# hasnainfarid/Mujoco_Gymnasium_Environments

Hardware: AMD Instinct MI355X
Metric: env steps/sec (whole node), humanoid_soccer 4096 envs/GPU at 1/2/4/8 MI355X (higher is better)
Workload: dtype f64

## Files before the change

### mujoco_gymnasium_environments_amd/csrc/mgx_api.hip

```cpp
#include <hip/hip_runtime.h>

#include <cmath>
#include <cstdio>
#include <cstring>
#include <map>
#include <mutex>
#include <string>
#include <vector>

#include "mgx_internal.h"

using namespace mgx;

MGX_PROF_SETTER(mgx_prof_set_buffer)

namespace {
thread_local std::string g_err;
int fail(int code, const std::string& msg) {
  g_err = msg;
  return code;
}
#define HIPCHK(x) MGX_HIPCHK(x)
}

// ... 493 lines not shown
  return pgs_lanes() == 64 ? a / 2 : a;
}

static int wide_arena_bytes(const mgx_model* m) {
  const int wide_lds = m->hooks.pgs_wide_lds;
  const int rb = m->precision == MGX_F32 ? 4 : 8;
  const int nv = m->precision == MGX_F32 ? m->mf.nv : m->md.nv;
  const int maxE = m->Ls.max_nefc;
  const int nbRun = (maxE / 4 + MGX_PGS_RING_LDS - 1) / MGX_PGS_RING_LDS * MGX_PGS_RING_LDS;
  const int nbA = nbRun + MGX_PGS_RING_LDS - 1;
  const int bcap = 32 + (maxE / 4) * (8 + 32 * ((nv + 7) / 8));
  const int worst = nbA * (4 * MGX_SCAL * rb + 4 * mgx_twl(false)) + ((bcap + 3) & ~3) * rb;
  return wide_lds && pgs_lanes() == 16 && worst + 64 <= 160 * 1024 ? (worst + 15) & ~15 : 0;
}

size_t mgx::make_staged_pipe(const mgx_model* m, void* ws, int n_env, int banks, Pipe* P, bool rk, int nobs) {
  int rb = m->precision == MGX_F32 ? 4 : 8;
  int nq = m->precision == MGX_F32 ? m->mf.nq : m->md.nq;
  int nv = m->precision == MGX_F32 ? m->mf.nv : m->md.nv;
  Pipe p{};
  p.base = (char*)ws;
  p.N = n_env; p.R = banks; p.S = n_env * (1 + banks);
  p.maxE = m->Ls.max_nefc; p.nv = nv; p.dpl = (nv + 7) / 8;
  const Hooks& H = m->hooks;
  const bool cap_env = H.pgs_lds_rows > 0;
  int capE = cap_env ? (H.pgs_lds_rows + 3) / 4 * 4 : MGX_PGS_LDS_ROWS;
  if (capE < 4 || capE > p.maxE) capE = MGX_PGS_LDS_ROWS;
  if (rk) {
    capE = H.rk_lds_rows > 0 ? (H.rk_lds_rows + 3) / 4 * 4 : 256;
    if (capE < 4) capE = 256;
  }
// ... 18 lines not shown
  p.bcap = 32 + (p.maxE / 4) * (8 + 32 * ((nv + 7) / 8));
  p.tw = MGX_TW;
  p.nobs = nobs;
  size_t off = 0;
  auto take = [&](size_t bytes) { size_t r = off; off = (off + bytes + 255) / 256 * 256; return r; };
  size_t S = (size_t)p.S, NB = (size_t)n_env * (banks > 0 ? banks : 1);
  p.o_ctr = take(64);
  p.o_carry = take(S * p.carry_stride * rb);
  p.o_carryi = take(S * p.carryi_stride * 4);
  p.o_ne = take(S * 4); p.o_blen = take(S * 4); p.o_niter = take(S * 4); p.o_k2list = take(S * 4); p.o_k2big = take(S * 4); p.o_fix = take((size_t)n_env * 4);
  p.hmain = !rk && !cap_env && !p.sqg && !H.pgs_lds_b && p.capE < p.maxE &&
            staged_pgs_lds_bytes(m, p.maxE, pgs_lanes(), 1, mgx_twl(false)) <=
                (H.pgs_wpc == 4 ? staged_pgs_lds_bytes(m, p.capE, pgs_lanes(), 0, mgx_twl(false))
                                : 160 * 1024 / H.pgs_wpc);
  if (p.hmain) p.warena = 0;
  p.prio_rows = H.pgs_prio_rows > 0 ? H.pgs_prio_rows : p.capE;
  p.nbk = (p.hmain ? p.maxE : p.capE) / 4 + 1;
  p.o_hist = take((size_t)(p.maxE / 4 + 1) * 4);
  p.o_blist = take((size_t)(p.maxE / 4 + 1) * S * 4);
  p.o_scal = take(S * p.maxE * MGX_SCAL * rb);
  p.o_blk = take(S * (p.maxE / 4) * p.tw * 4);
  p.o_B = take(S * (size_t)p.bcap * rb);
  p.o_vout = take(S * 64 * rb);
  p.o_bq = take(NB * nq * rb); p.o_bv = take(NB * nv * rb); p.o_ba = take(NB * nv * rb); p.o_btime = take(NB * rb);
  p.o_bobs = take(NB * nobs * 4); p.o_bprev = take(NB * 6 * rb); p.o_bwind = take(NB * 3 * rb);
  p.o_bk = take(NB * 4); p.o_bep = take(NB * 4); p.o_bwarn = take(NB * 4); p.o_bseed = take(NB * 8);
  int nb = m->precision == MGX_F32 ? m->mf.nbody : m->md.nbody;
  p.maxC = m->Ls.max_ncon;
  p.o_cpos = take(S * 3 * (size_t)p.maxC * rb);
  p.o_tq = take(nq * rb); p.o_tv = take(nv * rb); p.o_ta = take(64 * rb); p.o_tt = take(rb);
  p.o_tx = take(3 * nb * rb); p.o_txq = take(4 * nb * rb); p.o_tsc = take(3 * nb * rb); p.o_tn = take(4);
  p.o_tcg = take(2 * p.maxC * 4); p.o_tcd = take(p.maxC * rb); p.o_tcm = take(p.maxC * rb);
  p.o_rkw = take(S * 4);
  p.o_tscr = take(m->L.gB ? (size_t)m->L.gB_stride * rb : 64);
  if (rk) {
    const int nq4 = (nq + 3) & ~3;
    p.rk_stride = 2 * nq4 + 8 * 64 + 4;
    p.o_rk = take(S * p.rk_stride * rb);
    p.o_rks = take(S * 4);
  }
  if (P) *P = p;
  return off;
}
static size_t make_pipe(const mgx_model* m, void* ws, int n_env, int banks, Pipe* P) {
  return make_staged_pipe(m, ws, n_env, banks, P, false, 80);
}

int mgx::staged_pgs_lds_bytes(const mgx_model* m, int rows, int lps, int sqg, int twl) {
  int rb = m->precision == MGX_F32 ? 4 : 8;
  int nb3 = (rows / 4 + MGX_PGS_RING - 1) / MGX_PGS_RING * MGX_PGS_RING;
  const int spw = 64 / lps;
  const int sq = sqg ? 4 : 4 * MGX_SCAL;
  return spw * (sq * nb3 + 4) * rb + spw * nb3 * 4 * twl + 64;
}
static int pgs_lds_bytes(const mgx_model* m, int rows, int sqg = 0) {
  return staged_pgs_lds_bytes(m, rows, pgs_lanes(), sqg, mgx_twl(false));
}

mgx::Hooks mgx::read_hooks() {
  Hooks h;
  auto get = [](const char* name, int dflt) {
    const char* v = getenv(name);
    return v && *v ? atoi(v) : dflt;
  };
  h.pgs_lds_rows = get("MGX_PGS_LDS_ROWS", 0);
  h.rk_lds_rows = get("MGX_RK_LDS_ROWS", 0);
  h.pgs_single = get("MGX_PGS_SINGLE", 0);
  h.pgs_lds_b = get("MGX_PGS_LDS_B", MGX_PGS_LDS_B) != 0;
  h.pgs_arena = get("MGX_PGS_ARENA", 0);
  h.pgs_lds_pad = get("MGX_PGS_LDS_PAD", 0);
  h.pgs_wide_lds = get("MGX_PGS_WIDE_LDS", 1);
  h.pgs_spw = get("MGX_PGS_SPW", 0);
  h.pgs_prio_rows = get("MGX_PGS_PRIO_ROWS", 0);
  h.tight_bp = get("MGX_TIGHT_BROADPHASE", -1);
  h.pgs_wpc = get("MGX_PGS_WPC", 4);
  if (h.pgs_wpc < 4 || h.pgs_wpc > 16) h.pgs_wpc = 4;
  h.side_stream = get("MGX_SIDE_STREAM", 1) != 0;
  h.gcon = get("MGX_GCON", 1);
  h.rows_lds = get("MGX_ROWS_LDS", 0);
  return h;
}

struct SideStream {
  hipStream_t s;
  hipEvent_t rows, big;
};
static SideStream* side_stream(hipStream_t st) {
  static std::mutex mu;
// ... 28 lines not shown
                              float* obs, double* reward, uint8_t* terminated, uint8_t* truncated, float* final_obs,
                              int autoreset, uint64_t seed, int env_offset, int n_env, const uint8_t* mask,
                              hipStream_t st) {
  Pipe P;
  int banks = autoreset ? e->banks : 0;
  size_t need = make_pipe(m, e->workspace, n_env, e->banks, &P);
  if (e->workspace_bytes < need) return fail(MGX_E_ARG, "workspace smaller than mgx_soccer_workspace_bytes");
  int slots = n_env * (1 + banks);
  const Hooks& H = m->hooks;
  const int rlds = H.rows_lds > m->Ls.bytes && H.rows_lds <= 64 * 1024 ? H.rows_lds : m->Ls.bytes;
  launch_soccer_rows<T>(Ms, ids, *s, *e, action, n_env, mask, P, banks, slots, rlds, st);
  T scale = (T)1 / (M.meaninertia * (T)(M.nv > 1 ? M.nv : 1));
  const int wgrid = 64 / pgs_lanes() * MGX_PGS_WIDE_GRID, wlds = pgs_lds_bytes(m, P.maxE);
  int mlds = H.pgs_lds_b ? P.arena : pgs_lds_bytes(m, P.capE, P.sqg);
  if (P.hmain) mlds = std::max(mlds, pgs_lds_bytes(m, P.maxE, 1));
  if (H.pgs_lds_pad > mlds && H.pgs_lds_pad <= 96 * 1024) mlds = H.pgs_lds_pad;
  if (!H.pgs_lds_b && (P.maxE <= P.capE || P.hmain)) {
    launch_pgs<T>(P, slots, mlds, st, M.iterations, M.tolerance, scale, 0, H);
  } else if (SideStream* side = (!H.pgs_lds_b && H.side_stream) ? side_stream(st) : nullptr) {
    HIPCHK(hipEventRecord(side->rows, st));
    HIPCHK(hipStreamWaitEvent(side->s, side->rows, 0));
    launch_pgs<T>(P, wgrid, wlds, side->s, M.iterations, M.tolerance, scale, 1, H);
    HIPCHK(hipEventRecord(side->big, side->s));
    launch_pgs<T>(P, slots, mlds, st, M.iterations, M.tolerance, scale, 0, H);
    HIPCHK(hipStreamWaitEvent(st, side->big, 0));
  } else {
    launch_pgs<T>(P, slots, mlds, st, M.iterations, M.tolerance, scale, 0, H);
    launch_pgs<T>(P, wgrid, wlds, st, M.iterations, M.tolerance, scale, 1, H);
  }
  launch_soccer_finish<T>(Mf, ids, *s, *e, action, obs, reward, terminated, truncated, final_obs, autoreset, seed,
                          env_offset, n_env, mask, P, banks, m->Lf.bytes, st);
  int fgrid = n_env < 256 ? n_env : 256;
// ... 304 lines not shown
```

### mujoco_gymnasium_environments_amd/csrc/mgx_internal.h

```cpp
#pragma once
#include <hip/hip_runtime.h>

#include <string>

#include "../../include/mgx.h"
#include "mgx_bipedal.h"
#include "mgx_construction.h"
#include "mgx_dancing.h"
#include "mgx_martial.h"
#include "mgx_parkour.h"
#include "mgx_staged.h"

namespace mgx {
struct Hooks {
  int pgs_lds_rows = 0;
  int rk_lds_rows = 0;
  int pgs_single = 0;
  int pgs_lds_b = 0;
  int pgs_arena = 0;
  int pgs_lds_pad = 0;
  int pgs_wide_lds = 1;
  int pgs_spw = 0;
  int pgs_wpc = 4;
  int pgs_prio_rows = 0;
  int tight_bp = -1;
  int side_stream = 1;
  int gcon = 1;
  int rows_lds = 0;
};
Hooks read_hooks();
struct RayState;
struct SensorState;
}

struct mgx_model {
  mgx::Hooks hooks;
  int precision;
  int device;
  void* dbuf = nullptr;
// ... 58 lines not shown
template <typename T>
void launch_soccer_rows(const DevModel<T>& Ms, const SoccerIds<T>& ids, const mgx_state& s, const mgx_soccer_env& ev,
                        const float* action, int n_env, const uint8_t* mask, const Pipe& P, int banks, int slots, int lds,
                        hipStream_t st);
template <typename T>
void launch_soccer_finish(const DevModel<T>& Mf, const SoccerIds<T>& ids, const mgx_state& s, const mgx_soccer_env& ev,
                          const float* action, float* obs, double* reward, uint8_t* terminated, uint8_t* truncated,
                          float* final_obs, int autoreset, uint64_t seed, int env_offset, int n_env, const uint8_t* mask,
                          const Pipe& P, int banks, int lds, hipStream_t st);
template <typename T>
void launch_soccer_settle(const DevModel<T>& Ms, const DevModel<T>& Mf, const SoccerIds<T>& ids, const mgx_state& s,
                          const mgx_soccer_env& ev, const T* draws, float* obs, uint64_t seed, int env_offset, int n_env,
                          const uint8_t* mask, const Pipe& P, int mode, int grid, int lds, hipStream_t st, int maxit, T tol,
                          T scale);
int staged_kernels_configure(int precision, int ls, int lf, int settle);
size_t make_staged_pipe(const mgx_model* m, void* ws, int n_env, int banks, Pipe* P, bool rk, int nobs);
int staged_pgs_lds_bytes(const mgx_model* m, int rows, int lps, int sqg, int twl);
int bipedal_staged_configure(const mgx_model* m);
int bipedal_step_staged(const mgx_model* m, const mgx_state* s, const mgx_bipedal_env* e, const float* action, float* obs,
                        double* reward, uint8_t* terminated, uint8_t* truncated, float* final_obs, int autoreset,
                        uint64_t seed, int env_offset, int n_env, const uint8_t* mask, hipStream_t st);
int bipedal_reset_staged(const mgx_model* m, const mgx_state* s, const mgx_bipedal_env* e, const void* draws,
                         float* obs, uint64_t seed, int env_offset, int n_env, const uint8_t* mask, hipStream_t st);
int64_t bipedal_workspace_bytes(const mgx_model* m, int n_env, int banks);
int bipedal_workspace_init(const mgx_model* m, void* workspace, uint64_t bytes, int n_env, int banks, hipStream_t st);
bool parkour_staged_ok(const mgx_model* m);
int parkour_staged_configure(const mgx_model* m);
int parkour_step_staged(const mgx_model* m, const mgx_state* s, const mgx_parkour_env* e, const float* action, float* obs,
                        double* reward, uint8_t* terminated, uint8_t* truncated, float* final_obs, int autoreset,
                        uint64_t seed, int env_offset, int n_env, const uint8_t* mask, hipStream_t st);
int parkour_reset_staged(const mgx_model* m, const mgx_state* s, const mgx_parkour_env* e, const void* draws,
// ... 24 lines not shown
```

### mujoco_gymnasium_environments_amd/csrc/mgx_pk_staged.hip

```cpp
#include "mgx_internal.h"

using namespace mgx;

namespace mgx {

constexpr int PK_LPS = 16;
constexpr int PK_OBS = 95;
enum { PK_SETTLE_RESET = 0, PK_SETTLE_FIXUP = 1 };
enum { PK_SUBSTEPS = 10 };

template <typename T>
__device__ __forceinline__ void pk_bank_init_draws(const DevModel<T>& m, Env<T>& e, const ParkourIds<T>& ids,
                                                   const Pipe& P, int bi, int episode, uint64_t seed, T d0, T d1) {
  const int l = lane_id();
  reset_env(m, e);
  if (l == 0) {
    e.qpos[0] = (T)2.0; e.qpos[1] = (T)0.0; e.qpos[2] = (T)0.6;
    e.qpos[3] = (T)1; e.qpos[4] = 0; e.qpos[5] = 0; e.qpos[6] = 0;
    e.qpos[ids.platform_qpos] = d0;
    e.qpos[ids.pendulum_qpos] = d1;
  }
  wsync();
  copy_g(P.at<T>(P.o_bq) + (size_t)bi * m.nq, e.qpos, m.nq);
  if (l < m.nv) {
// ... 302 lines not shown
#define MGX_PK_EPL(EPL_VAR, CALL) \
  switch (EPL_VAR) {              \
    case 1: { constexpr int E = 1; CALL; } break; \
    case 2: { constexpr int E = 2; CALL; } break; \
    case 3: { constexpr int E = 3; CALL; } break; \
    default: { constexpr int E = 4; CALL; } break; \
  }

template <typename T>
int step_staged(const mgx_model* m, const DevModel<T>& M, const DevModel<T>& Ms, const DevModel<T>& Mf,
                const ParkourIds<T>& ids, const mgx_state* s, const mgx_parkour_env* e, const float* action,
                float* obs, double* reward, uint8_t* terminated, uint8_t* truncated, float* final_obs, int autoreset,
                uint64_t seed, int env_offset, int n_env, const uint8_t* mask, hipStream_t st) {
  Pipe P;
  const int banks = autoreset ? e->banks : 0;
  const size_t need = make_staged_pipe(m, e->workspace, n_env, e->banks, &P, false, PK_OBS);
  if (e->workspace_bytes < need) return fail(MGX_E_ARG, "workspace smaller than mgx_parkour_workspace_bytes");
  const int slots = n_env * (1 + banks);
  const T scale = (T)1 / (M.meaninertia * (T)(M.nv > 1 ? M.nv : 1));
  const int mlds = std::max(staged_pgs_lds_bytes(m, P.capE, PK_LPS, 0, 8),
                           P.hmain ? staged_pgs_lds_bytes(m, P.maxE, PK_LPS, 1, 8) : 0);
  const int spw = 64 / PK_LPS, grid = (slots + spw - 1) / spw;
  for (int k = 0; k < PK_SUBSTEPS; k++) {
    hipLaunchKernelGGL(k_pk_rows<T>, dim3(slots), dim3(64), m->Ls.bytes, st, Ms, ids, *s, action, e->action_f64, n_env,
                       mask, P, banks, k);
    MGX_PK_EPL(pk_epl(M), hipLaunchKernelGGL((k_pgs_groups<T, E, PK_LPS, false>), dim3(grid), dim3(64), mlds, st, P,
                                             M.iterations, M.tolerance, scale, spw, 0));
    if (banks && P.R > 0)
      hipLaunchKernelGGL(k_pk_bank_finish<T>, dim3(n_env * P.R), dim3(64), m->Lf.bytes, st, Mf, ids, n_env, P);
    hipLaunchKernelGGL(k_pk_finish<T>, dim3(n_env), dim3(64), m->Lf.bytes, st, Mf, ids, *s, *e, action, obs, reward,
                       terminated, truncated, final_obs, autoreset, seed, env_offset, n_env, mask, P, banks, k);
  }
  const int fgrid = n_env < 256 ? n_env : 256;
  MGX_PK_EPL(pk_epl(M), hipLaunchKernelGGL((k_pk_settle<T, E>), dim3(fgrid), dim3(64), pk_settle_lds(m, P), st, Ms, Mf,
                                           ids, *s, *e, (const T*)nullptr, obs, seed, env_offset, n_env,
                                           (const uint8_t*)nullptr, P, (int)PK_SETTLE_FIXUP, M.iterations, M.tolerance,
                                           scale));
  MGX_HIPCHK(hipGetLastError());
  return MGX_OK;
}

template <typename T>
int reset_staged(const mgx_model* m, const DevModel<T>& M, const DevModel<T>& Ms, const DevModel<T>& Mf,
                 const ParkourIds<T>& ids, const mgx_state* s, const mgx_parkour_env* e, const T* draws, float* obs,
                 uint64_t seed, int env_offset, int n_env, const uint8_t* mask, hipStream_t st) {
  Pipe P;
  const size_t need = make_staged_pipe(m, e->workspace, n_env, e->banks, &P, false, PK_OBS);
  if (e->workspace_bytes < need) return fail(MGX_E_ARG, "workspace smaller than mgx_parkour_workspace_bytes");
  const T scale = (T)1 / (M.meaninertia * (T)(M.nv > 1 ? M.nv : 1));
  MGX_PK_EPL(pk_epl(M), hipLaunchKernelGGL((k_pk_settle<T, E>), dim3(n_env), dim3(64), pk_settle_lds(m, P), st, Ms, Mf,
                                           ids, *s, *e, draws, obs, seed, env_offset, n_env, mask, P,
                                           (int)PK_SETTLE_RESET, M.iterations, M.tolerance, scale));
  MGX_HIPCHK(hipGetLastError());
  return MGX_OK;
}

template <typename T>
int configure_t(const mgx_model* m) {
  Pipe P;
  make_staged_pipe(m, nullptr, 1, 1, &P, false, PK_OBS);
  const int pl = staged_pgs_lds_bytes(m, P.maxE, PK_LPS, 0, 8);
  if (pl > 160 * 1024) return fail(MGX_E_CAPACITY, "staged parkour solver LDS exceeds 160 KiB");
  int rc = mgx_set_lds(k_pk_rows<T>, m->Ls.bytes) | mgx_set_lds(k_pk_finish<T>, m->Lf.bytes) |
           mgx_set_lds(k_pk_bank_finish<T>, m->Lf.bytes) | mgx_set_lds(k_pk_template<T, true>, m->L.bytes) |
           mgx_set_lds(k_pk_template<T, false>, m->L.bytes);
  const int sl = pk_settle_lds(m, P);
#define MGX_PK_SET(E) rc |= mgx_set_lds(k_pk_settle<T, E>, sl) | mgx_set_lds(k_pgs_groups<T, E, PK_LPS, false>, pl);
  MGX_PK_SET(1) MGX_PK_SET(2) MGX_PK_SET(3) MGX_PK_SET(4)
#undef MGX_PK_SET
  return rc;
}

}

namespace mgx {
bool parkour_staged_ok(const mgx_model* m) {
  const int nv = m->precision == MGX_F32 ? m->mf.nv : m->md.nv;
  if (!m->staged_ok || nv > 64 || pgs_lanes() != PK_LPS || m->hooks.pgs_lds_b) return false;
  Pipe P;
  make_staged_pipe(m, nullptr, 1, 1, &P, false, PK_OBS);
  return !P.sqg && (P.maxE <= P.capE || P.hmain);
}

int parkour_staged_configure(const mgx_model* m) {
  if (!parkour_staged_ok(m)) return MGX_OK;
  return m->precision == MGX_F32 ? configure_t<float>(m) : configure_t<double>(m);
}

int parkour_step_staged(const mgx_model* m, const mgx_state* s, const mgx_parkour_env* e, const float* action, float* obs,
                        double* reward, uint8_t* terminated, uint8_t* truncated, float* final_obs, int autoreset,
                        uint64_t seed, int env_offset, int n_env, const uint8_t* mask, hipStream_t st) {
  if (!parkour_staged_ok(m)) return fail(MGX_E_UNSUPPORTED, "staged parkour step: model outside the staged pipeline");
  if (e->banks < 0 || e->banks > 16) return fail(MGX_E_ARG, "banks must be in [0, 16]");
  if (m->precision == MGX_F32)
    return step_staged<float>(m, m->mf, m->mfs, m->mff, m->pkf, s, e, action, obs, reward, terminated, truncated,
                              final_obs, autoreset, seed, env_offset, n_env, mask, st);
// ... 3 lines not shown

int parkour_reset_staged(const mgx_model* m, const mgx_state* s, const mgx_parkour_env* e, const void* draws,
                         float* obs, uint64_t seed, int env_offset, int n_env, const uint8_t* mask, hipStream_t st) {
  if (!parkour_staged_ok(m)) return fail(MGX_E_UNSUPPORTED, "staged parkour step: model outside the staged pipeline");
  if (e->banks < 0 || e->banks > 16) return fail(MGX_E_ARG, "banks must be in [0, 16]");
  if (m->precision == MGX_F32)
    return reset_staged<float>(m, m->mf, m->mfs, m->mff, m->pkf, s, e, (const float*)draws, obs, seed, env_offset,
                               n_env, mask, st);
  return reset_staged<double>(m, m->md, m->mds, m->mdf, m->pkd, s, e, (const double*)draws, obs, seed, env_offset,
                              n_env, mask, st);
}

int64_t parkour_workspace_bytes(const mgx_model* m, int n_env, int banks) {
  if (!m || n_env <= 0 || banks < 0 || banks > 16) return fail(MGX_E_ARG, "bad argument");
  if (!parkour_staged_ok(m)) return fail(MGX_E_UNSUPPORTED, "staged parkour step: model outside the staged pipeline");
  return (int64_t)make_staged_pipe(m, nullptr, n_env, banks, nullptr, false, PK_OBS);
}

int parkour_workspace_init(const mgx_model* m, void* workspace, uint64_t bytes, int n_env, int banks, hipStream_t st) {
  if (!m || !workspace || n_env <= 0 || banks < 0 || banks > 16) return fail(MGX_E_ARG, "bad argument");
  if (!parkour_staged_ok(m)) return fail(MGX_E_UNSUPPORTED, "staged parkour step: model outside the staged pipeline");
  Pipe P;
  const size_t need = make_staged_pipe(m, workspace, n_env, banks, &P, false, PK_OBS);
  if (bytes < need) return fail(MGX_E_ARG, "workspace smaller than mgx_parkour_workspace_bytes");
  MGX_HIPCHK(hipMemsetAsync(workspace, 0, need, st));
  const size_t nb = (size_t)n_env * (banks > 0 ? banks : 1);
  MGX_HIPCHK(hipMemsetAsync(P.base + P.o_bk, 0xFF, nb * 4, st));
  if (m->precision == MGX_F32) {
    if (m->L.gB) hipLaunchKernelGGL((k_pk_template<float, true>), dim3(1), dim3(64), m->L.bytes, st, m->mf, P);
    else hipLaunchKernelGGL((k_pk_template<float, false>), dim3(1), dim3(64), m->L.bytes, st, m->mf, P);
  } else {
    if (m->L.gB) hipLaunchKernelGGL((k_pk_template<double, true>), dim3(1), dim3(64), m->L.bytes, st, m->md, P);
    else hipLaunchKernelGGL((k_pk_template<double, false>), dim3(1), dim3(64), m->L.bytes, st, m->md, P);
  }
  MGX_HIPCHK(hipGetLastError());
  return MGX_OK;
}
}
// ... 1 lines not shown
```

### mujoco_gymnasium_environments_amd/csrc/mgx_staged.h

```cpp
#pragma once
#include "mgx_soccer.h"

namespace mgx {

#define MGX_SCAL 5
#define MGX_SQ(k, i) (4 * (k) + (i))
#define MGX_TW 4
__host__ __device__ constexpr int mgx_twl(bool dofb) { return dofb ? 4 : 8; }
#define MGX_PGS_LPS 16
#define MGX_PGS_LDS_B 0
#define MGX_PGS_RING 2
#define MGX_PGS_RING_LDS 2
#define MGX_PGS_LDS_ROWS 192
#define MGX_PGS_WIDE_GRID 256
#define MGX_PGS_WIDE_LDS_GRID 32
#define MGX_PGS_ARENA_F64 49152
#define MGX_PGS_ARENA_F32 32768
enum { FIX_RESET = 2 };

struct Pipe {
  char* base;
  int N, R, S, maxE, dpl, nv;
  int carry_stride;
  int carryi_stride;
  int bcap;
  int capE;
  int arena;
  int sqg;
  int prio_rows;
  int hmain;
  int warena;
  size_t o_cpos;
  size_t o_carry, o_carryi, o_ne, o_blen, o_niter, o_k2list, o_k2big, o_ctr, o_fix, o_scal, o_blk, o_B, o_vout;
  int nbk;
  size_t o_hist, o_blist;
  size_t o_bq, o_bv, o_ba, o_btime, o_bobs, o_bprev, o_bwind, o_bk, o_bep, o_bwarn, o_bseed;
  size_t o_tq, o_tv, o_ta, o_tt, o_tx, o_txq, o_tsc, o_tn, o_tcg, o_tcd, o_tcm;
  int maxC;
  int tw;
  int nobs;
  int rk_stride;
  size_t o_rk, o_rks, o_rkw, o_tscr;
  template <typename X> __device__ __forceinline__ X* at(size_t off) const { return reinterpret_cast<X*>(base + off); }
  __device__ __forceinline__ int* ctr() const { return at<int>(o_ctr); }
};
// ... 380 lines not shown
  for (int k = l; k < 2 * e.ncon; k += 64) ci[k] = e.con_geom[k];
  int* cx = ci + m.L.carry_ints;
  if (l == 0) {
    cx[0] = e.ncon; cx[1] = ne; cx[2] = e.overflow; cx[3] = warn;
    P.at<int>(P.o_ne)[slot] = ne;
    P.at<int>(P.o_blen)[slot] = boff;
#ifdef MGX_PROFILE
    if (g_mgx_prof && slot < (int)gridDim.x) {
      g_mgx_prof[slot * 32 + 20] += ne;
      g_mgx_prof[slot * 32 + 22] += e.ncon;
      g_mgx_prof[slot * 32 + 23] += 1;
      if ((unsigned long long)ne > g_mgx_prof[slot * 32 + 24]) g_mgx_prof[slot * 32 + 24] = ne;
      g_mgx_prof[slot * 32 + 25] += e.overflow != 0;
    }
#endif
    if (!list_slot) {
    } else if (ne > P.capE && !P.hmain) {
      int idx = atomicAdd(P.ctr() + 2, 1);
      P.at<int>(P.o_k2big)[idx] = slot;
    } else if (ne > 0) {
      int idx = atomicAdd(P.ctr() + 1, 1);
      P.at<int>(P.o_k2list)[idx] = slot;
      const int nb = ne >> 2;
      const int r = atomicAdd(P.at<int>(P.o_hist) + nb, 1);
      P.at<int>(P.o_blist)[(size_t)nb * P.S + r] = slot;
    }
  }
}

template <int CTRL>
__device__ __forceinline__ float dpp_row(float v) {
  return __builtin_bit_cast(float, __builtin_amdgcn_mov_dpp(__builtin_bit_cast(int, v), CTRL, 0xf, 0xf, true));
// ... 57 lines not shown
      t.g[d] = in ? e.x + 8u + 4u * (uint32_t)__popcll(below) : 0u;
    }
  } else {
    const uint32_t* e = bt + 8 * blk;
    t.a = e[0];
#pragma unroll
    for (int d = 0; d < EPL; d++) {
      const int gi = d * (LPS / 8) + (j >> 3);
      t.g[d] = (gi < 7 ? e[1 + gi] : 0u) + 4u * (uint32_t)(j & 7);
    }
  }
}

typedef float mgx_f2 __attribute__((ext_vector_type(2)));

template <typename T, int EPL, int LPS, int FS>
__device__ __forceinline__ void pgs_load_block(PgsBlk<T, EPL>& k, const T* Bsl, const T* sq, const T* fb,
                                               const PgsTab<EPL>& t, int blk, int sblk, int j) {
  typedef typename Vec4T<T>::type V4;
  const V4* pa = reinterpret_cast<const V4*>(Bsl + t.a);
  k.a0 = pa[0];
  k.a1 = pa[1];
#pragma unroll
  for (int d = 0; d < EPL; d++) k.b[d] = *reinterpret_cast<const V4*>(Bsl + t.g[d]);
  const V4* q = reinterpret_cast<const V4*>(sq + 4 * MGX_SCAL * sblk);
  k.qb = q[0];
  k.qf = *reinterpret_cast<const V4*>(fb + FS * blk);
  k.qR = q[2];
  k.qi = q[3];
  k.qh = q[4];
  __builtin_amdgcn_sched_barrier(0);
}
template <typename T, int EPL, int LPS, int FS, bool DOFB>
__device__ __forceinline__ void pgs_load_block(PgsBlk<T, EPL>& k, const T* Bsl, const T* sq, const T* fb,
                                               const uint32_t* bt, int blk, int sblk, int j) {
  PgsTab<EPL> t;
  pgs_load_tab<EPL, LPS, DOFB>(t, bt, blk, j);
  pgs_load_block<T, EPL, LPS, FS>(k, Bsl, sq, fb, t, blk, sblk, j);
}
// ... 18 lines not shown
  }
  d0 = p01.x; d1 = p01.y; d2 = p23.x; d3 = p23.y;
}

template <typename T, int EPL>
__device__ __forceinline__ void pgs_update(const PgsBlk<T, EPL>& k, T (&v)[EPL], T dl0, T dl1, T dl2, T dl3) {
#pragma unroll
  for (int d = 0; d < EPL; d++) {
    T x = fma(dl0, k.b[d].x, v[d]);
    x = fma(dl1, k.b[d].y, x);
    x = fma(dl2, k.b[d].z, x);
    v[d] = fma(dl3, k.b[d].w, x);
  }
}

template <typename T, int EPL, int LPS>
__device__ __forceinline__ void pgs_block(const PgsBlk<T, EPL>& k, T (&v)[EPL], T* fblk, bool ok0, T& impr) {
  typedef typename Vec4T<T>::type V4;
  V4* qf = reinterpret_cast<V4*>(fblk);
  const V4 qb = k.qb, f = k.qf, qR = k.qR, qi = k.qi, qh = k.qh;
  T d0, d1, d2, d3;
  pgs_dots(k, v, d0, d1, d2, d3);
  const T t0 = qb.x + qR.x * f.x, t1 = qb.y + qR.y * f.y;
  const T t2 = qb.z + qR.z * f.z, t3 = qb.w + qR.w * f.w;
  slot_sum4<LPS>(d0, d1, d2, d3);
  T dl0, dl1, dl2, dl3;
  V4 nfv;
#define MGX_PGS_ROW(C, I, DOT, DL)                                \
  {                                                               \
    const T fr = f.C, ai = qi.C, hd = qh.C;                       \
    T res = (DOT) + t##I;                                         \
    T fn = fmax(fr - res * ai, (T)0);                             \
    T delta = fn - fr;                                            \
    T change = delta * (delta * hd + res);                        \
    bool keep = !ok0 || change > (T)1e-10;                        \
    DL = keep ? (T)0 : delta;                                     \
    impr -= keep ? (T)0 : change;                                 \
    nfv.C = keep ? fr : fn;                                       \
  }
  MGX_PGS_ROW(x, 0, d0, dl0)
  MGX_PGS_ROW(y, 1, d1 + k.a0.x * dl0, dl1)
  MGX_PGS_ROW(z, 2, d2 + k.a0.y * dl0 + k.a0.z * dl1, dl2)
  MGX_PGS_ROW(w, 3, d3 + k.a0.w * dl0 + k.a1.x * dl1 + k.a1.y * dl2, dl3)
#undef MGX_PGS_ROW
  if ((lane_id() & (LPS - 1)) == 0) *qf = nfv;
  pgs_update(k, v, dl0, dl1, dl2, dl3);
}

template <typename T, int EPL, int LPS, bool BLDS, bool SQG = false, bool DOFB = false>
__device__ __forceinline__ void pgs_group(const Pipe& P, char* smem, int slot, int capE, int maxit, T tol, T scale,
                                          int spw, int arena = -1) {
  constexpr int RING = BLDS ? MGX_PGS_RING_LDS : MGX_PGS_RING;
  typedef typename Vec4T<T>::type V4;
  constexpr int SPW = 64 / LPS;
  const int l = threadIdx.x, s = l / LPS, j = l % LPS;
  (void)spw;
  const int ne = slot >= 0 ? P.at<int>(P.o_ne)[slot] : 0;
  const int nblk = ne >> 2;
  int nm = nblk;
  nm = max(nm, __shfl_xor(nm, 8));
  nm = max(nm, __shfl_xor(nm, 16));
  nm = max(nm, __shfl_xor(nm, 32));
  int nbMax = __builtin_amdgcn_readfirstlane(nm);
  if (spw < 0) nbMax = capE / 4;
  const int nbRun = (nbMax + RING - 1) / RING * RING;
  const size_t sl = (size_t)(slot >= 0 ? slot : 0);
  const T* gsc = P.at<T>(P.o_scal) + sl * P.maxE * MGX_SCAL;
  constexpr int TWL = mgx_twl(DOFB);
  const uint32_t* gbt = P.at<uint32_t>(P.o_blk) + sl * (P.maxE / 4) * MGX_TW;
  const uint16_t* gbt16 = reinterpret_cast<const uint16_t*>(gbt);
// ... 25 lines not shown
      if (arena < 0 && j == 0 && slot >= 0) P.at<int>(P.o_k2big)[atomicAdd(P.ctr() + 2, 1)] = slot;
      return;
    }
    sc = reinterpret_cast<T*>(smem + off);
    bt = reinterpret_cast<uint32_t*>(sc + 4 * MGX_SCAL * nbA);
    T* Bs = reinterpret_cast<T*>(bt + TWL * nbA);
    for (int q = 4 * j; q < blen; q += 4 * LPS)
      *reinterpret_cast<V4*>(Bs + q) = *reinterpret_cast<const V4*>(gB + q);
    Bsl = Bs;
    sq = sc;
    fb = sc + MGX_SQ(1, 0);
    for (int q = j; q < MGX_SCAL * 4 * nbA; q += LPS) sc[q] = q < ne * MGX_SCAL ? gsc[q] : (T)0;
  } else {
    const int nbcap = capE / 4;
    nbA = (nbcap + RING - 1) / RING * RING;
    const int sstride = (SG ? 4 : 4 * MGX_SCAL) * nbA + 4;
    sc = reinterpret_cast<T*>(smem) + s * sstride;
    bt = reinterpret_cast<uint32_t*>(reinterpret_cast<T*>(smem) + SPW * sstride) + s * TWL * nbA;
    Bsl = gB;
    if constexpr (SG) {
      sq = gsc;
      fb = sc;
      for (int q = j; q < 4 * nbA; q += LPS) sc[q] = q < ne ? gsc[(q >> 2) * (4 * MGX_SCAL) + MGX_SQ(1, q & 3)] : (T)0;
    } else {
      sq = sc;
      fb = sc + MGX_SQ(1, 0);
      for (int q = j; q < MGX_SCAL * 4 * nbA; q += LPS) sc[q] = q < ne * MGX_SCAL ? gsc[q] : (T)0;
    }
  }
  const int sbmax = P.maxE / 4 - 1;
  for (int q = j; q < TWL * nbA; q += LPS) bt[q] = q < TWL * nblk ? (DOFB ? gbt[q] : (uint32_t)gbt16[q]) : 0u;
  __syncthreads();
  T v[EPL];
#pragma unroll
  for (int d = 0; d < EPL; d++) v[d] = 0;
  for (int b = 0; b < nbMax; b++) {
    PgsBlk<T, EPL> k;
    pgs_load_block<T, EPL, LPS, FS, DOFB>(k, Bsl, sq, fb, bt, b, min(b, sbmax), j);
    const T* qf = fb + FS * b;
    bool ok = b < nblk;
    T f0 = ok ? qf[0] : (T)0, f1 = ok ? qf[1] : (T)0, f2 = ok ? qf[2] : (T)0, f3 = ok ? qf[3] : (T)0;
    pgs_update(k, v, f0, f1, f2, f3);
  }
  T cpart = 0;
  for (int b = 0; b < nbMax; b++) {
    PgsBlk<T, EPL> k;
// ... 6 lines not shown
      const T* qq = sq + 4 * b * MGX_SCAL;
      const T* qf = fb + FS * b;
#pragma unroll
      for (int i = 0; i < 4; i++) {
        const T fi = qf[i];
        cpart += fi * (qq[MGX_SQ(0, i)] + (T)0.5 * (dd[i] + qq[MGX_SQ(2, i)] * fi));
      }
    }
  }
  if (cpart > 0) {
    for (int r = j; r < ne; r += LPS) fb[(r >> 2) * FS + (r & 3)] = 0;
#pragma unroll
    for (int d = 0; d < EPL; d++) v[d] = 0;
  }
  __syncthreads();
  bool act = ne > 0;
  int it = 0;
#ifdef MGX_PROFILE
  unsigned long long t_sweep0 = __builtin_amdgcn_s_memtime();
  unsigned long long r_sweep0 = __builtin_amdgcn_s_memrealtime();
  int nsweep = 0;
#endif
  for (int iter = 0; iter < maxit; iter++) {
    if (__ballot(act) == 0ull) break;
#ifdef MGX_PROFILE
    nsweep++;
#endif
    T impr = 0;
    PgsBlk<T, EPL> R[RING];
    PgsTab<EPL> tn;
    pgs_load_tab<EPL, LPS, DOFB>(tn, bt, 0, j);
#pragma unroll
    for (int k = 0; k < RING - 1; k++) {
      pgs_load_block<T, EPL, LPS, FS>(R[k], Bsl, sq, fb, tn, k, min(k, sbmax), j);
      pgs_load_tab<EPL, LPS, DOFB>(tn, bt, k + 1, j);
    }
    for (int b0 = 0; b0 < nbRun; b0 += RING) {
#pragma unroll
      for (int k = 0; k < RING; k++) {
        const int bn = min(b0 + k + RING - 1, nbA - 1);
        pgs_load_block<T, EPL, LPS, FS>(R[(k + RING - 1) % RING], Bsl, sq, fb, tn, bn, min(bn, sbmax), j);
        pgs_load_tab<EPL, LPS, DOFB>(tn, bt, min(bn + 1, nbA - 1), j);
        pgs_block<T, EPL, LPS>(R[k], v, fb + FS * (b0 + k), act && b0 + k < nblk, impr);
      }
    }
    if (act) {
      it++;
      if (impr * scale < tol) act = false;
    }
  }
#ifdef MGX_PROFILE
  if (g_mgx_prof && l == 0) {
    unsigned long long* pr = g_mgx_prof + (size_t)blockIdx.x * 32;
    pr[26] += __builtin_amdgcn_s_memtime() - t_sweep0;
    pr[27] += (unsigned long long)nsweep * nbMax;
    pr[28] += 1;
    pr[29] += __builtin_amdgcn_s_memrealtime() - r_sweep0;
    if ((unsigned long long)(nsweep * nbMax) > pr[30]) pr[30] = nsweep * nbMax;
  }
#endif
  if (slot >= 0) {
    T* vo = P.at<T>(P.o_vout) + (size_t)slot * 64;
#pragma unroll
    for (int d = 0; d < EPL; d++)
      {
        const int dof = 8 * (d * (LPS / 8) + (j >> 3)) + (j & 7);
        if (dof < P.nv) vo[dof] = v[d];
      }
    if (j == 0) P.at<int>(P.o_niter)[slot] = it;
  }
}

__device__ __forceinline__ int sorted_slot(const Pipe& P, int idx, int LPS) {
  const int* hist = P.at<int>(P.o_hist);
  const int* bl = P.at<int>(P.o_blist);
  const int l = lane_id();
// ... 9 lines not shown
    }
    for (int q = 0; q < 64; q += LPS) {
      const int iq = __shfl(idx, q);
      const unsigned long long m = __ballot(iq >= 0 && acc + x > iq);
      if (m) {
        const int f = __ffsll((long long)m) - 1;
        const int xf = __shfl(x, f), hf = __shfl(h, f);
        const int rank = iq - (acc + xf - hf);
        const int sq = bl[(size_t)(top - f) * P.S + rank];
        if (l >= q && l < q + LPS && slot < 0) slot = sq;
      }
    }
    acc += __shfl(x, 63);
  }
  return slot;
}

template <typename T, int EPL, int LPS, bool BLDS, bool SQG = false, bool DOFB = false>
__global__ void __launch_bounds__(64) k_pgs_groups(Pipe P, int maxit, T tol, T scale, int spw, int big) {
  extern __shared__ __attribute__((aligned(16))) char smem[];
  if (!big && blockIdx.x == 0 && threadIdx.x == 0) P.ctr()[0] = 0;
  const int cnt = P.ctr()[big ? 2 : 1];
  const int* list = P.at<int>(P.o_k2big);
  const int spn = spw < 0 ? -spw : spw;
  const int s = threadIdx.x / LPS;
  if (big) __builtin_amdgcn_s_setprio(3);
  const bool dup = big && BLDS;
  for (int base = blockIdx.x * spn; base < cnt; base += gridDim.x * spn) {
    const int idx = dup ? base : (s < spn && base + s < cnt) ? base + s : -1;
    const int slot = big ? (idx >= 0 ? list[idx] : -1) : sorted_slot(P, idx, LPS);
    if constexpr (!BLDS && !SQG) {
      if (!big) {
        int nm = slot >= 0 ? P.at<int>(P.o_ne)[slot] : 0;
        nm = max(nm, __shfl_xor(nm, 16));
        nm = max(nm, __shfl_xor(nm, 32));
        nm = __builtin_amdgcn_readfirstlane(nm);
        const bool hi = nm > P.prio_rows;
        if (hi) __builtin_amdgcn_s_setprio(3);
        if (P.hmain && nm > P.capE) {
          pgs_group<T, EPL, LPS, false, true, DOFB>(P, smem, slot, P.maxE, maxit, tol, scale, spw, -1);
          if (hi) __builtin_amdgcn_s_setprio(0);
          __syncthreads();
          continue;
// ... 282 lines not shown
```

Before: 1.640 million.

## Split PGS solve of large-constraint envs across all 64 lanes of a wave

```diff
diff --git a/mujoco_gymnasium_environments_amd/csrc/mgx_api.hip b/mujoco_gymnasium_environments_amd/csrc/mgx_api.hip
--- a/mujoco_gymnasium_environments_amd/csrc/mgx_api.hip
+++ b/mujoco_gymnasium_environments_amd/csrc/mgx_api.hip
@@ -531,7 +531,8 @@
   return wide_lds && pgs_lanes() == 16 && worst + 64 <= 160 * 1024 ? (worst + 15) & ~15 : 0;
 }
 
-size_t mgx::make_staged_pipe(const mgx_model* m, void* ws, int n_env, int banks, Pipe* P, bool rk, int nobs) {
+size_t mgx::make_staged_pipe(const mgx_model* m, void* ws, int n_env, int banks, Pipe* P, bool rk, int nobs,
+                             int split_default) {
   int rb = m->precision == MGX_F32 ? 4 : 8;
   int nq = m->precision == MGX_F32 ? m->mf.nq : m->md.nq;
   int nv = m->precision == MGX_F32 ? m->mf.nv : m->md.nv;
@@ -580,8 +581,21 @@
                 (H.pgs_wpc == 4 ? staged_pgs_lds_bytes(m, p.capE, pgs_lanes(), 0, mgx_twl(false))
                                 : 160 * 1024 / H.pgs_wpc);
   if (p.hmain) p.warena = 0;
+  p.split_blocks = 0;
+  const int split = H.pgs_split_blocks >= 0 ? H.pgs_split_blocks : split_default;
+  if (!rk && !p.sqg && !H.pgs_lds_b && pgs_lanes() == 16 && split > 0) {
+    const int one = staged_pgs_lds_bytes(m, p.maxE, 64, 0, mgx_twl(false));
+    int main_lds = staged_pgs_lds_bytes(m, p.capE, 16, 0, mgx_twl(false));
+    if (p.hmain) main_lds = std::max(main_lds, staged_pgs_lds_bytes(m, p.maxE, 16, 1, mgx_twl(false)));
+    const bool b32 = (uint64_t)p.bcap * (uint64_t)rb < (1ull << 32);
+    if (b32 && one <= (cap_env ? 160 * 1024 : main_lds)) {
+      p.split_blocks = std::min(split, p.capE / 4 + 1);
+      p.hmain = 0;
+      p.warena = 0;
+    }
+  }
   p.prio_rows = H.pgs_prio_rows > 0 ? H.pgs_prio_rows : p.capE;
-  p.nbk = (p.hmain ? p.maxE : p.capE) / 4 + 1;
+  p.nbk = (p.hmain || p.split_blocks ? p.maxE : p.capE) / 4 + 1;
   p.o_hist = take((size_t)(p.maxE / 4 + 1) * 4);
   p.o_blist = take((size_t)(p.maxE / 4 + 1) * S * 4);
   p.o_scal = take(S * p.maxE * MGX_SCAL * rb);
@@ -609,7 +623,7 @@
   return off;
 }
 static size_t make_pipe(const mgx_model* m, void* ws, int n_env, int banks, Pipe* P) {
-  return make_staged_pipe(m, ws, n_env, banks, P, false, 80);
+  return make_staged_pipe(m, ws, n_env, banks, P, false, 80, MGX_PGS_SPLIT_BLOCKS);
 }
 
 int mgx::staged_pgs_lds_bytes(const mgx_model* m, int rows, int lps, int sqg, int twl) {
@@ -638,6 +652,7 @@
   h.pgs_wide_lds = get("MGX_PGS_WIDE_LDS", 1);
   h.pgs_spw = get("MGX_PGS_SPW", 0);
   h.pgs_prio_rows = get("MGX_PGS_PRIO_ROWS", 0);
+  h.pgs_split_blocks = get("MGX_PGS_SPLIT_BLOCKS", -1);
   h.tight_bp = get("MGX_TIGHT_BROADPHASE", -1);
   h.pgs_wpc = get("MGX_PGS_WPC", 4);
   if (h.pgs_wpc < 4 || h.pgs_wpc > 16) h.pgs_wpc = 4;
@@ -696,8 +711,9 @@
   const int wgrid = 64 / pgs_lanes() * MGX_PGS_WIDE_GRID, wlds = pgs_lds_bytes(m, P.maxE);
   int mlds = H.pgs_lds_b ? P.arena : pgs_lds_bytes(m, P.capE, P.sqg);
   if (P.hmain) mlds = std::max(mlds, pgs_lds_bytes(m, P.maxE, 1));
+  if (P.split_blocks) mlds = std::max(mlds, staged_pgs_lds_bytes(m, P.maxE, 64, 0, mgx_twl(false)));
   if (H.pgs_lds_pad > mlds && H.pgs_lds_pad <= 96 * 1024) mlds = H.pgs_lds_pad;
-  if (!H.pgs_lds_b && (P.maxE <= P.capE || P.hmain)) {
+  if (!H.pgs_lds_b && (P.maxE <= P.capE || P.hmain || P.split_blocks)) {
     launch_pgs<T>(P, slots, mlds, st, M.iterations, M.tolerance, scale, 0, H);
   } else if (SideStream* side = (!H.pgs_lds_b && H.side_stream) ? side_stream(st) : nullptr) {
     HIPCHK(hipEventRecord(side->rows, st));
diff --git a/mujoco_gymnasium_environments_amd/csrc/mgx_internal.h b/mujoco_gymnasium_environments_amd/csrc/mgx_internal.h
--- a/mujoco_gymnasium_environments_amd/csrc/mgx_internal.h
+++ b/mujoco_gymnasium_environments_amd/csrc/mgx_internal.h
@@ -23,6 +23,7 @@
   int pgs_spw = 0;
   int pgs_wpc = 4;
   int pgs_prio_rows = 0;
+  int pgs_split_blocks = -1;
   int tight_bp = -1;
   int side_stream = 1;
   int gcon = 1;
@@ -111,7 +112,8 @@
                           const uint8_t* mask, const Pipe& P, int mode, int grid, int lds, hipStream_t st, int maxit, T tol,
                           T scale);
 int staged_kernels_configure(int precision, int ls, int lf, int settle);
-size_t make_staged_pipe(const mgx_model* m, void* ws, int n_env, int banks, Pipe* P, bool rk, int nobs);
+size_t make_staged_pipe(const mgx_model* m, void* ws, int n_env, int banks, Pipe* P, bool rk, int nobs,
+                        int split_default = 0);
 int staged_pgs_lds_bytes(const mgx_model* m, int rows, int lps, int sqg, int twl);
 int bipedal_staged_configure(const mgx_model* m);
 int bipedal_step_staged(const mgx_model* m, const mgx_state* s, const mgx_bipedal_env* e, const float* action, float* obs,
diff --git a/mujoco_gymnasium_environments_amd/csrc/mgx_pk_staged.hip b/mujoco_gymnasium_environments_amd/csrc/mgx_pk_staged.hip
--- a/mujoco_gymnasium_environments_amd/csrc/mgx_pk_staged.hip
+++ b/mujoco_gymnasium_environments_amd/csrc/mgx_pk_staged.hip
@@ -6,6 +6,7 @@
 
 constexpr int PK_LPS = 16;
 constexpr int PK_OBS = 95;
+constexpr int PK_SPLIT_BLOCKS = 56;
 enum { PK_SETTLE_RESET = 0, PK_SETTLE_FIXUP = 1 };
 enum { PK_SUBSTEPS = 10 };
 
@@ -340,12 +341,13 @@
                 uint64_t seed, int env_offset, int n_env, const uint8_t* mask, hipStream_t st) {
   Pipe P;
   const int banks = autoreset ? e->banks : 0;
-  const size_t need = make_staged_pipe(m, e->workspace, n_env, e->banks, &P, false, PK_OBS);
+  const size_t need = make_staged_pipe(m, e->workspace, n_env, e->banks, &P, false, PK_OBS, PK_SPLIT_BLOCKS);
   if (e->workspace_bytes < need) return fail(MGX_E_ARG, "workspace smaller than mgx_parkour_workspace_bytes");
   const int slots = n_env * (1 + banks);
   const T scale = (T)1 / (M.meaninertia * (T)(M.nv > 1 ? M.nv : 1));
-  const int mlds = std::max(staged_pgs_lds_bytes(m, P.capE, PK_LPS, 0, 8),
-                           P.hmain ? staged_pgs_lds_bytes(m, P.maxE, PK_LPS, 1, 8) : 0);
+  const int mlds = std::max({staged_pgs_lds_bytes(m, P.capE, PK_LPS, 0, 8),
+                            P.hmain ? staged_pgs_lds_bytes(m, P.maxE, PK_LPS, 1, 8) : 0,
+                            P.split_blocks ? staged_pgs_lds_bytes(m, P.maxE, 64, 0, 8) : 0});
   const int spw = 64 / PK_LPS, grid = (slots + spw - 1) / spw;
   for (int k = 0; k < PK_SUBSTEPS; k++) {
     hipLaunchKernelGGL(k_pk_rows<T>, dim3(slots), dim3(64), m->Ls.bytes, st, Ms, ids, *s, action, e->action_f64, n_env,
@@ -371,7 +373,7 @@
                  const ParkourIds<T>& ids, const mgx_state* s, const mgx_parkour_env* e, const T* draws, float* obs,
                  uint64_t seed, int env_offset, int n_env, const uint8_t* mask, hipStream_t st) {
   Pipe P;
-  const size_t need = make_staged_pipe(m, e->workspace, n_env, e->banks, &P, false, PK_OBS);
+  const size_t need = make_staged_pipe(m, e->workspace, n_env, e->banks, &P, false, PK_OBS, PK_SPLIT_BLOCKS);
   if (e->workspace_bytes < need) return fail(MGX_E_ARG, "workspace smaller than mgx_parkour_workspace_bytes");
   const T scale = (T)1 / (M.meaninertia * (T)(M.nv > 1 ? M.nv : 1));
   MGX_PK_EPL(pk_epl(M), hipLaunchKernelGGL((k_pk_settle<T, E>), dim3(n_env), dim3(64), pk_settle_lds(m, P), st, Ms, Mf,
@@ -384,7 +386,7 @@
 template <typename T>
 int configure_t(const mgx_model* m) {
   Pipe P;
-  make_staged_pipe(m, nullptr, 1, 1, &P, false, PK_OBS);
+  make_staged_pipe(m, nullptr, 1, 1, &P, false, PK_OBS, PK_SPLIT_BLOCKS);
   const int pl = staged_pgs_lds_bytes(m, P.maxE, PK_LPS, 0, 8);
   if (pl > 160 * 1024) return fail(MGX_E_CAPACITY, "staged parkour solver LDS exceeds 160 KiB");
   int rc = mgx_set_lds(k_pk_rows<T>, m->Ls.bytes) | mgx_set_lds(k_pk_finish<T>, m->Lf.bytes) |
@@ -404,8 +406,8 @@
   const int nv = m->precision == MGX_F32 ? m->mf.nv : m->md.nv;
   if (!m->staged_ok || nv > 64 || pgs_lanes() != PK_LPS || m->hooks.pgs_lds_b) return false;
   Pipe P;
-  make_staged_pipe(m, nullptr, 1, 1, &P, false, PK_OBS);
-  return !P.sqg && (P.maxE <= P.capE || P.hmain);
+  make_staged_pipe(m, nullptr, 1, 1, &P, false, PK_OBS, PK_SPLIT_BLOCKS);
+  return !P.sqg && (P.maxE <= P.capE || P.hmain || P.split_blocks);
 }
 
 int parkour_staged_configure(const mgx_model* m) {
@@ -439,14 +441,14 @@
 int64_t parkour_workspace_bytes(const mgx_model* m, int n_env, int banks) {
   if (!m || n_env <= 0 || banks < 0 || banks > 16) return fail(MGX_E_ARG, "bad argument");
   if (!parkour_staged_ok(m)) return fail(MGX_E_UNSUPPORTED, "staged parkour step: model outside the staged pipeline");
-  return (int64_t)make_staged_pipe(m, nullptr, n_env, banks, nullptr, false, PK_OBS);
+  return (int64_t)make_staged_pipe(m, nullptr, n_env, banks, nullptr, false, PK_OBS, PK_SPLIT_BLOCKS);
 }
 
 int parkour_workspace_init(const mgx_model* m, void* workspace, uint64_t bytes, int n_env, int banks, hipStream_t st) {
   if (!m || !workspace || n_env <= 0 || banks < 0 || banks > 16) return fail(MGX_E_ARG, "bad argument");
   if (!parkour_staged_ok(m)) return fail(MGX_E_UNSUPPORTED, "staged parkour step: model outside the staged pipeline");
   Pipe P;
-  const size_t need = make_staged_pipe(m, workspace, n_env, banks, &P, false, PK_OBS);
+  const size_t need = make_staged_pipe(m, workspace, n_env, banks, &P, false, PK_OBS, PK_SPLIT_BLOCKS);
   if (bytes < need) return fail(MGX_E_ARG, "workspace smaller than mgx_parkour_workspace_bytes");
   MGX_HIPCHK(hipMemsetAsync(workspace, 0, need, st));
   const size_t nb = (size_t)n_env * (banks > 0 ? banks : 1);
diff --git a/mujoco_gymnasium_environments_amd/csrc/mgx_staged.h b/mujoco_gymnasium_environments_amd/csrc/mgx_staged.h
--- a/mujoco_gymnasium_environments_amd/csrc/mgx_staged.h
+++ b/mujoco_gymnasium_environments_amd/csrc/mgx_staged.h
@@ -12,6 +12,7 @@
 #define MGX_PGS_RING 2
 #define MGX_PGS_RING_LDS 2
 #define MGX_PGS_LDS_ROWS 192
+#define MGX_PGS_SPLIT_BLOCKS 40
 #define MGX_PGS_WIDE_GRID 256
 #define MGX_PGS_WIDE_LDS_GRID 32
 #define MGX_PGS_ARENA_F64 49152
@@ -29,6 +30,7 @@
   int sqg;
   int prio_rows;
   int hmain;
+  int split_blocks;
   int warena;
   size_t o_cpos;
   size_t o_carry, o_carryi, o_ne, o_blen, o_niter, o_k2list, o_k2big, o_ctr, o_fix, o_scal, o_blk, o_B, o_vout;
@@ -439,8 +441,9 @@
       g_mgx_prof[slot * 32 + 25] += e.overflow != 0;
     }
 #endif
+    if (list_slot && ne > P.capE) atomicAdd(P.ctr() + 7, 1);
     if (!list_slot) {
-    } else if (ne > P.capE && !P.hmain) {
+    } else if (ne > P.capE && !P.hmain && !P.split_blocks) {
       int idx = atomicAdd(P.ctr() + 2, 1);
       P.at<int>(P.o_k2big)[idx] = slot;
     } else if (ne > 0) {
@@ -528,15 +531,20 @@
 
 typedef float mgx_f2 __attribute__((ext_vector_type(2)));
 
-template <typename T, int EPL, int LPS, int FS>
+template <bool U32, typename T>
+__device__ __forceinline__ const T* pgs_b_at(const T* Bsl, uint32_t entry) {
+  if constexpr (U32) return reinterpret_cast<const T*>(reinterpret_cast<const char*>(Bsl) + entry * (uint32_t)sizeof(T));
+  else return Bsl + entry;
+}
+template <typename T, int EPL, int LPS, int FS, bool U32 = false>
 __device__ __forceinline__ void pgs_load_block(PgsBlk<T, EPL>& k, const T* Bsl, const T* sq, const T* fb,
                                                const PgsTab<EPL>& t, int blk, int sblk, int j) {
   typedef typename Vec4T<T>::type V4;
-  const V4* pa = reinterpret_cast<const V4*>(Bsl + t.a);
+  const V4* pa = reinterpret_cast<const V4*>(pgs_b_at<U32>(Bsl, t.a));
   k.a0 = pa[0];
   k.a1 = pa[1];
 #pragma unroll
-  for (int d = 0; d < EPL; d++) k.b[d] = *reinterpret_cast<const V4*>(Bsl + t.g[d]);
+  for (int d = 0; d < EPL; d++) k.b[d] = *reinterpret_cast<const V4*>(pgs_b_at<U32>(Bsl, t.g[d]));
   const V4* q = reinterpret_cast<const V4*>(sq + 4 * MGX_SCAL * sblk);
   k.qb = q[0];
   k.qf = *reinterpret_cast<const V4*>(fb + FS * blk);
@@ -585,16 +593,66 @@
   }
 }
 
-template <typename T, int EPL, int LPS>
-__device__ __forceinline__ void pgs_block(const PgsBlk<T, EPL>& k, T (&v)[EPL], T* fblk, bool ok0, T& impr) {
+template <typename T, int EPL>
+struct PgsRow {
+  T b[EPL];
+};
+template <typename T, int EPL>
+__device__ __forceinline__ void pgs_load_row(PgsRow<T, EPL>& r, const T* Bsl, uint32_t g, const PgsTab<EPL>& t) {
+#pragma unroll
+  for (int d = 0; d < EPL; d++) r.b[d] = *pgs_b_at<true>(Bsl, t.g[d] + g);
+}
+template <int EPL>
+__device__ __forceinline__ double pgs_row_dot(const PgsRow<double, EPL>& r, const double (&v)[EPL]) {
+  double x = 0;
+#pragma unroll
+  for (int d = 0; d < EPL; d++) x += r.b[d] * v[d];
+  return x;
+}
+template <int EPL>
+__device__ __forceinline__ float pgs_row_dot(const PgsRow<float, EPL>& r, const float (&v)[EPL]) {
+  float x = 0.f;
+#pragma unroll
+  for (int d = 0; d < EPL; d++) x = __builtin_fmaf(r.b[d], v[d], x);
+  return x;
+}
+template <int LPS>
+__device__ __forceinline__ float oct_sum(float x) {
+  x += dpp_row<0xB1>(x);
+  x += dpp_row<0x4E>(x);
+  x += dpp_row<0x141>(x);
+  if constexpr (LPS == 16) x += dpp_row<0x140>(x);
+  return x;
+}
+template <int L>
+__device__ __forceinline__ float lane_value(float x) {
+  return __builtin_bit_cast(float, __builtin_amdgcn_readlane(__builtin_bit_cast(int, x), L));
+}
+template <int L>
+__device__ __forceinline__ double lane_value(double x) {
+  const uint64_t u = __builtin_bit_cast(uint64_t, x);
+  const uint32_t lo = (uint32_t)__builtin_amdgcn_readlane((int)(uint32_t)u, L);
+  const uint32_t hi = (uint32_t)__builtin_amdgcn_readlane((int)(uint32_t)(u >> 32), L);
+  return __builtin_bit_cast(double, (uint64_t)lo | ((uint64_t)hi << 32));
+}
+
+template <typename T, int EPL, int LPS, bool SPLIT = false>
+__device__ __forceinline__ void pgs_block(const PgsBlk<T, EPL>& k, T (&v)[EPL], T* fblk, bool ok0, T& impr,
+                                          const PgsRow<T, EPL>* row = nullptr) {
   typedef typename Vec4T<T>::type V4;
   V4* qf = reinterpret_cast<V4*>(fblk);
   const V4 qb = k.qb, f = k.qf, qR = k.qR, qi = k.qi, qh = k.qh;
   T d0, d1, d2, d3;
-  pgs_dots(k, v, d0, d1, d2, d3);
+  if constexpr (SPLIT) d0 = pgs_row_dot(*row, v);
+  else pgs_dots(k, v, d0, d1, d2, d3);
   const T t0 = qb.x + qR.x * f.x, t1 = qb.y + qR.y * f.y;
   const T t2 = qb.z + qR.z * f.z, t3 = qb.w + qR.w * f.w;
-  slot_sum4<LPS>(d0, d1, d2, d3);
+  if constexpr (SPLIT) {
+    const T dg = oct_sum<LPS>(d0);
+    d0 = lane_value<0>(dg); d1 = lane_value<LPS>(dg); d2 = lane_value<2 * LPS>(dg); d3 = lane_value<3 * LPS>(dg);
+  } else {
+    slot_sum4<LPS>(d0, d1, d2, d3);
+  }
   T dl0, dl1, dl2, dl3;
   V4 nfv;
 #define MGX_PGS_ROW(C, I, DOT, DL)                                \
@@ -614,17 +672,20 @@
   MGX_PGS_ROW(z, 2, d2 + k.a0.y * dl0 + k.a0.z * dl1, dl2)
   MGX_PGS_ROW(w, 3, d3 + k.a0.w * dl0 + k.a1.x * dl1 + k.a1.y * dl2, dl3)
 #undef MGX_PGS_ROW
-  if ((lane_id() & (LPS - 1)) == 0) *qf = nfv;
+  if ((lane_id() & ((SPLIT ? 64 : LPS) - 1)) == 0) *qf = nfv;
   pgs_update(k, v, dl0, dl1, dl2, dl3);
 }
 
-template <typename T, int EPL, int LPS, bool BLDS, bool SQG = false, bool DOFB = false>
+template <typename T, int EPL, int LPS, bool BLDS, bool SQG = false, bool DOFB = false, bool SPLIT = false>
 __device__ __forceinline__ void pgs_group(const Pipe& P, char* smem, int slot, int capE, int maxit, T tol, T scale,
                                           int spw, int arena = -1) {
   constexpr int RING = BLDS ? MGX_PGS_RING_LDS : MGX_PGS_RING;
   typedef typename Vec4T<T>::type V4;
-  constexpr int SPW = 64 / LPS;
-  const int l = threadIdx.x, s = l / LPS, j = l % LPS;
+  static_assert(!SPLIT || (!BLDS && !SQG && !DOFB && LPS == 16), "row-split mode: the 16-lane global-B solver");
+  constexpr int SPW = SPLIT ? 1 : 64 / LPS;
+  constexpr int FL = SPLIT ? 64 : LPS;
+  const int l = threadIdx.x, j = l % LPS;
+  const int s = SPLIT ? 0 : l / LPS, fj = SPLIT ? l : j;
   (void)spw;
   const int ne = slot >= 0 ? P.at<int>(P.o_ne)[slot] : 0;
   const int nblk = ne >> 2;
@@ -680,6 +741,7 @@
   } else {
     const int nbcap = capE / 4;
     nbA = (nbcap + RING - 1) / RING * RING;
+    if constexpr (SPLIT) nbA = min(nbA, nbRun + RING - 1);
     const int sstride = (SG ? 4 : 4 * MGX_SCAL) * nbA + 4;
     sc = reinterpret_cast<T*>(smem) + s * sstride;
     bt = reinterpret_cast<uint32_t*>(reinterpret_cast<T*>(smem) + SPW * sstride) + s * TWL * nbA;
@@ -691,11 +753,11 @@
     } else {
       sq = sc;
       fb = sc + MGX_SQ(1, 0);
-      for (int q = j; q < MGX_SCAL * 4 * nbA; q += LPS) sc[q] = q < ne * MGX_SCAL ? gsc[q] : (T)0;
+      for (int q = fj; q < MGX_SCAL * 4 * nbA; q += FL) sc[q] = q < ne * MGX_SCAL ? gsc[q] : (T)0;
     }
   }
   const int sbmax = P.maxE / 4 - 1;
-  for (int q = j; q < TWL * nbA; q += LPS) bt[q] = q < TWL * nblk ? (DOFB ? gbt[q] : (uint32_t)gbt16[q]) : 0u;
+  for (int q = fj; q < TWL * nbA; q += FL) bt[q] = q < TWL * nblk ? (DOFB ? gbt[q] : (uint32_t)gbt16[q]) : 0u;
   __syncthreads();
   T v[EPL];
 #pragma unroll
@@ -732,6 +794,8 @@
     for (int d = 0; d < EPL; d++) v[d] = 0;
   }
   __syncthreads();
+  const uint32_t grow = (uint32_t)(l / LPS);
+  (void)grow;
   bool act = ne > 0;
   int it = 0;
 #ifdef MGX_PROFILE
@@ -746,20 +810,23 @@
 #endif
     T impr = 0;
     PgsBlk<T, EPL> R[RING];
+    PgsRow<T, EPL> W[RING];
     PgsTab<EPL> tn;
     pgs_load_tab<EPL, LPS, DOFB>(tn, bt, 0, j);
 #pragma unroll
     for (int k = 0; k < RING - 1; k++) {
-      pgs_load_block<T, EPL, LPS, FS>(R[k], Bsl, sq, fb, tn, k, min(k, sbmax), j);
+      if constexpr (SPLIT) pgs_load_row(W[k], Bsl, grow, tn);
+      pgs_load_block<T, EPL, LPS, FS, SPLIT>(R[k], Bsl, sq, fb, tn, k, min(k, sbmax), j);
       pgs_load_tab<EPL, LPS, DOFB>(tn, bt, k + 1, j);
     }
     for (int b0 = 0; b0 < nbRun; b0 += RING) {
 #pragma unroll
       for (int k = 0; k < RING; k++) {
         const int bn = min(b0 + k + RING - 1, nbA - 1);
-        pgs_load_block<T, EPL, LPS, FS>(R[(k + RING - 1) % RING], Bsl, sq, fb, tn, bn, min(bn, sbmax), j);
+        if constexpr (SPLIT) pgs_load_row(W[(k + RING - 1) % RING], Bsl, grow, tn);
+        pgs_load_block<T, EPL, LPS, FS, SPLIT>(R[(k + RING - 1) % RING], Bsl, sq, fb, tn, bn, min(bn, sbmax), j);
         pgs_load_tab<EPL, LPS, DOFB>(tn, bt, min(bn + 1, nbA - 1), j);
-        pgs_block<T, EPL, LPS>(R[k], v, fb + FS * (b0 + k), act && b0 + k < nblk, impr);
+        pgs_block<T, EPL, LPS, SPLIT>(R[k], v, fb + FS * (b0 + k), act && b0 + k < nblk, impr, &W[k]);
       }
     }
     if (act) {
@@ -777,7 +844,7 @@
     if ((unsigned long long)(nsweep * nbMax) > pr[30]) pr[30] = nsweep * nbMax;
   }
 #endif
-  if (slot >= 0) {
+  if (slot >= 0 && (!SPLIT || l < LPS)) {
     T* vo = P.at<T>(P.o_vout) + (size_t)slot * 64;
 #pragma unroll
     for (int d = 0; d < EPL; d++)
@@ -817,6 +884,14 @@
     acc += __shfl(x, 63);
   }
   return slot;
+}
+__device__ __forceinline__ int split_count(const Pipe& P) {
+  const int* hist = P.at<int>(P.o_hist);
+  int x = 0;
+  for (int b = P.split_blocks + lane_id(); b < P.nbk; b += 64) x += hist[b];
+#pragma unroll
+  for (int o = 32; o >= 1; o >>= 1) x += __shfl_xor(x, o);
+  return __builtin_amdgcn_readfirstlane(x);
 }
 
 template <typename T, int EPL, int LPS, bool BLDS, bool SQG = false, bool DOFB = false>
@@ -829,7 +904,27 @@
   const int s = threadIdx.x / LPS;
   if (big) __builtin_amdgcn_s_setprio(3);
   const bool dup = big && BLDS;
-  for (int base = blockIdx.x * spn; base < cnt; base += gridDim.x * spn) {
+  constexpr bool CAN_SPLIT = !BLDS && !SQG && !DOFB && LPS == 16;
+  int K = 0;
+  if constexpr (CAN_SPLIT) {
+    if (!big && P.split_blocks > 0) K = min(split_count(P), cnt);
+  }
+  const int nw = K + (cnt - K + spn - 1) / spn;
+  for (int w = blockIdx.x; w < nw; w += gridDim.x) {
+    if constexpr (CAN_SPLIT) {
+      if (w < K) {
+        const int slot = __builtin_amdgcn_readfirstlane(sorted_slot(P, w, LPS));
+        const int ne = slot >= 0 ? P.at<int>(P.o_ne)[slot] : 0;
+        const bool hi = ne > P.prio_rows;
+        if (hi) __builtin_amdgcn_s_setprio(3);
+        pgs_group<T, EPL, LPS, false, false, false, true>(P, smem, slot, P.maxE, maxit, tol, scale, spw, -1);
+        if (hi) __builtin_amdgcn_s_setprio(0);
+        if (ne > P.capE && threadIdx.x == 0) atomicAdd(P.ctr() + 6, 1);
+        __syncthreads();
+        continue;
+      }
+    }
+    const int base = K + (w - K) * spn;
     const int idx = dup ? base : (s < spn && base + s < cnt) ? base + s : -1;
     const int slot = big ? (idx >= 0 ? list[idx] : -1) : sorted_slot(P, idx, LPS);
     if constexpr (!BLDS && !SQG) {
```

After: 1.722 million, median of 6. +5.0%, better.
